# jinbeizame007/pytorch-r2d2-DPG

Measured on NVIDIA H100. Metric: learner sequence-steps/sec (batch x seq_len), higher is better.
Workload: dtype bf16x3 (fp32 operands split into bf16 hi+lo, three tensor-core passes, fp32 accumulate: ~16-bit operands)

## Files before the change

pytorch-r2d2-dpg_b200/csrc/lstm_scan.cu:

```cuda
#include <cooperative_groups.h>
#include <stdlib.h>

#include "gemm.cuh"
#include "lstm_scan.cuh"
#include "elementwise.cuh"
#include "sm90.cuh"

namespace cg = cooperative_groups;

namespace r2d2 {
namespace {

constexpr int SCAN_THREADS = 256;
constexpr int UNITS_PER_CTA = 32;
constexpr int ROWS_PER_CTA = 128;
constexpr int GT_LD = ROWS_PER_CTA + 4;
constexpr int DG_LD = ROWS_PER_CTA + 8;
constexpr unsigned long long kWaitLimitNs = 4000000000ull;

__device__ unsigned g_scan_status = 0;

__device__ __forceinline__ float accurate_sigmoid(float x) { return 1.0f / (1.0f + expf(-x)); }

__device__ __forceinline__ unsigned long long global_ns() {
  unsigned long long t;
  asm volatile("mov.u64 %0, %globaltimer;" : "=l"(t));
  return t;
}

__device__ __forceinline__ void wait_slice(uint64_t* bar, uint32_t parity) {
  if (sm90::mbar_try_wait(bar, parity)) return;
  if (*reinterpret_cast<volatile unsigned*>(&g_scan_status)) return;
  const unsigned long long t0 = global_ns();
  while (!sm90::mbar_try_wait(bar, parity)) {
    if (global_ns() - t0 > kWaitLimitNs) {
      atomicExch(&g_scan_status, 1u);
      return;
    }
  }
}

__device__ __forceinline__ uint32_t slice_parity(int s) { return (uint32_t)((s - 1) >> 1) & 1u; }

template <int H> __host__ __device__ constexpr bool w_hi_in_smem() { return H > 256; }

template <int H, int NB>
struct FwdSmem {
  static constexpr int C = H / 32;
  static constexpr int HROW = UNITS_PER_CTA + 8;
  static constexpr int SLICE = 2 * NB * HROW;
  static constexpr int W_BYTES = w_hi_in_smem<H>() ? (H / 16) * 8 * 32 * 16 : 0;
  static constexpr int HB_ELEMS = 2 * C * SLICE;
  static constexpr int GT_ELEMS = NB * GT_LD;
  static constexpr int HS_ELEMS = SLICE;
  static constexpr int BAR_OFF = W_BYTES + HB_ELEMS * 2 + GT_ELEMS * 4 + HS_ELEMS * 2;
  static constexpr int BYTES = BAR_OFF + 2 * C * 8;
  static_assert((SLICE * 2) % 16 == 0 && BAR_OFF % 16 == 0, "bulk copies need 16-byte granules");
  static_assert(BYTES <= 232448, "forward scan tile does not fit in 227 KB of shared memory");
};

template <int H, int NB>
__global__ void __launch_bounds__(SCAN_THREADS, 1) lstm_scan_fwd_kernel(ScanFwdParams p) {
  constexpr int C = H / 32, KS = H / 16, NT = NB / 8;
  constexpr bool WS = w_hi_in_smem<H>();
  using SM = FwdSmem<H, NB>;
  constexpr int HROW = SM::HROW, SLICE = SM::SLICE;
  cg::cluster_group cluster = cg::this_cluster();
  const int rank = (int)cluster.block_rank();
  const int b0 = (blockIdx.x / C) * NB;
  const int tid = threadIdx.x, lane = tid & 31, w = tid >> 5;
  const int g = lane >> 2, c = lane & 3;
  const int B = p.B, S = p.T * p.repeat;

  extern __shared__ __align__(16) unsigned char smem_raw[];
  uint4* w_hi_s = reinterpret_cast<uint4*>(smem_raw);
  __nv_bfloat16* hb = reinterpret_cast<__nv_bfloat16*>(smem_raw + SM::W_BYTES);
  float* gt = reinterpret_cast<float*>(smem_raw + SM::W_BYTES + SM::HB_ELEMS * 2);
  __nv_bfloat16* hstage = reinterpret_cast<__nv_bfloat16*>(smem_raw + SM::W_BYTES + SM::HB_ELEMS * 2 + SM::GT_ELEMS * 4);
  uint64_t* bar = reinterpret_cast<uint64_t*>(smem_raw + SM::BAR_OFF);

  for (int idx = tid; idx < NB * H; idx += SCAN_THREADS) {
    const int n = idx / H, k = idx % H, b = b0 + n;
    float v = (b < B && p.h0) ? __ldg(p.h0 + (size_t)b * H + k) : 0.f;
    __nv_bfloat16 hi, lo;
    split_bf16(v, hi, lo);
    __nv_bfloat16* row = hb + (0 * C + k / UNITS_PER_CTA) * SLICE + n * HROW + k % UNITS_PER_CTA;
    row[0] = hi;
    row[NB * HROW] = lo;
  }
  const int ug = rank * 32 + lane;
  float cst[NT];
#pragma unroll
  for (int e = 0; e < NT; ++e) {
    const int b = b0 + w + 8 * e;
    cst[e] = 0.f;
    if (b < B) {
      float hv = p.h0 ? __ldg(p.h0 + (size_t)b * H + ug) : 0.f;
      float cv = p.c0 ? __ldg(p.c0 + (size_t)b * H + ug) : 0.f;
      p.hs[(size_t)b * H + ug] = hv;
      p.cs[(size_t)b * H + ug] = cv;
      cst[e] = cv;
    }
  }
  if (tid < 2 * C) {
    sm90::mbar_init(bar + tid, 1);
    sm90::fence_mbar_init_cluster();
    sm90::mbar_arrive_expect_tx(bar + tid, SLICE * 2);
  }

  uint32_t a_hi[WS ? 1 : KS][4], a_lo[KS][4];
  {
    const int gate = w >> 1;
    const int u_lo = (w & 1) * 16 + g;
    const float* w_r0 = p.whh + (size_t)(gate * H + rank * 32 + u_lo) * H;
    const float* w_r1 = w_r0 + (size_t)8 * H;
#pragma unroll
    for (int ks = 0; ks < KS; ++ks) {
      const int k = ks * 16 + 2 * c;
      float2 v0 = __ldg(reinterpret_cast<const float2*>(w_r0 + k));
      float2 v1 = __ldg(reinterpret_cast<const float2*>(w_r1 + k));
      float2 v2 = __ldg(reinterpret_cast<const float2*>(w_r0 + k + 8));
      float2 v3 = __ldg(reinterpret_cast<const float2*>(w_r1 + k + 8));
      uint32_t h[4];
      split_pack2(v0.x, v0.y, h[0], a_lo[ks][0]);
      split_pack2(v1.x, v1.y, h[1], a_lo[ks][1]);
      split_pack2(v2.x, v2.y, h[2], a_lo[ks][2]);
      split_pack2(v3.x, v3.y, h[3], a_lo[ks][3]);
      if constexpr (WS) {
        w_hi_s[(ks * 8 + w) * 32 + lane] = make_uint4(h[0], h[1], h[2], h[3]);
      } else {
#pragma unroll
        for (int f = 0; f < 4; ++f) a_hi[ks][f] = h[f];
      }
    }
  }
  __syncthreads();
  cluster.sync();

  const size_t gstride = (size_t)4 * H;
  for (int s = 0; s < S; ++s) {
    const int cur = s & 1, nxt = cur ^ 1;
    const int t = s / p.repeat;

#pragma unroll
    for (int nt = 0; nt < NT; ++nt)
#pragma unroll
      for (int f = 0; f < 4; ++f) {
        const int n = nt * 8 + 2 * c + (f & 1), r = 16 * w + g + (f >> 1) * 8, b = b0 + n;
        if (b < B) sm90::cp_async_4(gt + n * GT_LD + r, p.gin + ((size_t)t * B + b) * gstride + (r >> 5) * H + rank * 32 + (r & 31));
      }
    sm90::cp_async_commit();

    float acc[NT][4];
#pragma unroll
    for (int nt = 0; nt < NT; ++nt)
#pragma unroll
      for (int e = 0; e < 4; ++e) acc[nt][e] = 0.f;
    const __nv_bfloat16* hb_cur = hb + cur * C * SLICE;
    uint64_t* bar_cur = bar + cur * C;
    const uint32_t parity = slice_parity(s);
#pragma unroll
    for (int ks = 0; ks < KS; ++ks) {
      if ((ks & 1) == 0 && s > 0) wait_slice(bar_cur + ks / 2, parity);
      const __nv_bfloat16* hb_hi = hb_cur + (ks / 2) * SLICE;
      const __nv_bfloat16* hb_lo = hb_hi + NB * HROW;
      uint32_t ah[4];
      if constexpr (WS) {
        const uint4 v = w_hi_s[(ks * 8 + w) * 32 + lane];
        ah[0] = v.x; ah[1] = v.y; ah[2] = v.z; ah[3] = v.w;
      } else {
#pragma unroll
        for (int f = 0; f < 4; ++f) ah[f] = a_hi[ks][f];
      }
#pragma unroll
      for (int nt = 0; nt < NT; ++nt) {
        const int off = (nt * 8 + g) * HROW + (ks & 1) * 16 + 2 * c;
        uint32_t bh[2], bl[2];
        bh[0] = *reinterpret_cast<const uint32_t*>(hb_hi + off);
        bh[1] = *reinterpret_cast<const uint32_t*>(hb_hi + off + 8);
        bl[0] = *reinterpret_cast<const uint32_t*>(hb_lo + off);
        bl[1] = *reinterpret_cast<const uint32_t*>(hb_lo + off + 8);
        mma_bf16_16816(acc[nt], a_lo[ks], bh);
        mma_bf16_16816(acc[nt], ah, bl);
        mma_bf16_16816(acc[nt], ah, bh);
      }
    }
    sm90::cp_async_wait_all();
#pragma unroll
    for (int nt = 0; nt < NT; ++nt) {
      const int n = nt * 8 + 2 * c, r = 16 * w + g;
      gt[n * GT_LD + r] += acc[nt][0];
      gt[(n + 1) * GT_LD + r] += acc[nt][1];
      gt[n * GT_LD + r + 8] += acc[nt][2];
      gt[(n + 1) * GT_LD + r + 8] += acc[nt][3];
    }
    if (w == 0 && lane < C) sm90::bulk_wait_read_all();
    __syncthreads();
    if (s > 0 && tid < C) sm90::mbar_arrive_expect_tx(bar_cur + tid, SLICE * 2);

#pragma unroll
    for (int e = 0; e < NT; ++e) {
      const int n = w + 8 * e, b = b0 + n;
      __nv_bfloat16 hi = __float2bfloat16_rn(0.f), lo = hi;
      if (b < B) {
        const float* gr = gt + n * GT_LD + lane;
        const float ig = accurate_sigmoid(gr[0]);
        const float fg = accurate_sigmoid(gr[32]);
        const float gg = tanhf(gr[64]);
        const float og = accurate_sigmoid(gr[96]);
        const float cn = fg * cst[e] + ig * gg;
        const float hn = og * tanhf(cn);
        cst[e] = cn;
        if (!p.no_save) {
          float* go = p.gates + ((size_t)s * B + b) * gstride + ug;
          go[0] = ig; go[H] = fg; go[2 * H] = gg; go[3 * H] = og;
          p.cs[((size_t)(s + 1) * B + b) * H + ug] = cn;
        }
        p.hs[((size_t)(s + 1) * B + b) * H + ug] = hn;
        if (p.head_in && (s % p.repeat) == p.repeat - 1)
          p.head_in[((size_t)t * B + b) * H + ug] = tanhf(hn);
        split_bf16(hn, hi, lo);
      }
      hstage[(0 * NB + n) * HROW + lane] = hi;
      hstage[(1 * NB + n) * HROW + lane] = lo;
    }
    sm90::fence_proxy_async_smem();
    __syncthreads();

    if (s + 1 < S && w == 0 && lane < C) {
      const uint32_t slot = sm90::smem_u32(hb + (nxt * C + rank) * SLICE);
      const uint32_t slot_bar = sm90::smem_u32(bar + nxt * C + rank);
      sm90::bulk_copy_s2cluster(sm90::map_cluster(slot, lane), sm90::smem_u32(hstage), SLICE * 2,
                                sm90::map_cluster(slot_bar, lane));
      sm90::bulk_commit();
    }
  }
  cluster.sync();
}

template <int H, int NB>
struct BwdSmem {
  static constexpr int C = H / 32;
  static constexpr int DG_ELEMS = 2 * NB * DG_LD;
  static constexpr int PS_LD = NB + 2;
  static constexpr int PS_ELEMS = 2 * C * UNITS_PER_CTA * PS_LD;
  static constexpr int PS_BYTES_PER_SRC = UNITS_PER_CTA * NB * 4;
  static constexpr int MT = (H / 16 + 7) / 8;
  static constexpr int W_BYTES = w_hi_in_smem<H>() ? MT * 8 * 8 * 32 * 16 : 0;
  static constexpr int STAGE_PLANES = 6;
  static constexpr int STAGE_ELEMS = STAGE_PLANES * NB * UNITS_PER_CTA;
  static constexpr int BAR_OFF = W_BYTES + DG_ELEMS * 2 + PS_ELEMS * 4 + STAGE_ELEMS * 4;
  static constexpr int BYTES = BAR_OFF + 2 * C * 8;
  static_assert(BAR_OFF % 8 == 0, "mbarrier alignment");
  static_assert(BYTES <= 232448, "BPTT scan tile does not fit in 227 KB of shared memory");
};

template <int H, int NB>
__global__ void __launch_bounds__(SCAN_THREADS, 1) lstm_scan_bwd_kernel(ScanBwdParams p) {
  constexpr int C = H / 32, NT = NB / 8;
  constexpr int M_TILES = H / 16;
  constexpr int MT = (M_TILES + 7) / 8;
  constexpr int KS = ROWS_PER_CTA / 16;
  constexpr bool WS = w_hi_in_smem<H>();
  using SM = BwdSmem<H, NB>;
  cg::cluster_group cluster = cg::this_cluster();
  const int rank = (int)cluster.block_rank();
  const int b0 = (blockIdx.x / C) * NB;
  const int tid = threadIdx.x, lane = tid & 31, w = tid >> 5;
  const int g = lane >> 2, c = lane & 3;
  const int B = p.B, S = p.T * p.repeat;

  extern __shared__ __align__(16) unsigned char smem_raw[];
  uint4* w_hi_s = reinterpret_cast<uint4*>(smem_raw);
  __nv_bfloat16* dgs = reinterpret_cast<__nv_bfloat16*>(smem_raw + SM::W_BYTES);
  float* ps = reinterpret_cast<float*>(smem_raw + SM::W_BYTES + SM::DG_ELEMS * 2);
  float* stage = ps + SM::PS_ELEMS;
  uint64_t* bar = reinterpret_cast<uint64_t*>(smem_raw + SM::BAR_OFF);
  constexpr int PLANE = NB * UNITS_PER_CTA;
  constexpr size_t gstride = (size_t)4 * H;

  auto head_step = [&](int s) {
    const int rel = s - p.head_first_step;
    return p.dh_head && rel >= 0 && (rel % p.repeat) == p.repeat - 1;
  };
  auto prefetch = [&](int s) {
    const int rel = s - p.head_first_step;
    const bool head = head_step(s);
    unsigned tv;
    asm volatile("mov.u32 %0, %%tid.x;" : "=r"(tv));
    const int lane = tv & 31, w = tv >> 5, ug = rank * 32 + lane;
#pragma unroll
    for (int e = 0; e < NT; ++e) {
      const int n = w + 8 * e, b = b0 + n;
      if (b < B) {
        float* st = stage + n * UNITS_PER_CTA + lane;
        const float* gs = p.gates + ((size_t)s * B + b) * gstride + ug;
#pragma unroll
        for (int q = 0; q < 4; ++q) sm90::cp_async_4(st + q * PLANE, gs + q * H);
        sm90::cp_async_4(st + 4 * PLANE, p.cs + ((size_t)s * B + b) * H + ug);
        if (head) sm90::cp_async_4(st + 5 * PLANE, p.dh_head + ((size_t)(rel / p.repeat) * B + b) * H + ug);
      }
    }
    sm90::cp_async_commit();
  };

  if (tid < 2 * C) {
    sm90::mbar_init(bar + tid, 1);
    sm90::fence_mbar_init_cluster();
    sm90::mbar_arrive_expect_tx(bar + tid, SM::PS_BYTES_PER_SRC);
  }
  prefetch(S - 1);

  const float* w_t = p.whh + (size_t)(rank * 32 + 2 * c) * H + w * MT * 16 + g;
  uint32_t a_hi[WS ? 1 : MT][WS ? 1 : KS][4], a_lo[MT][KS][4];
#pragma unroll
  for (int i = 0; i < MT; ++i) {
    const int mi = w * MT + i;
#pragma unroll
    for (int ks = 0; ks < KS; ++ks) {
      uint32_t h[4];
#pragma unroll
      for (int f = 0; f < 4; ++f) {
        float v0 = 0.f, v1 = 0.f;
        if (mi < M_TILES) {
          const float* w0 = w_t + ((ks >> 1) * H + (ks & 1) * 16 + (f >> 1) * 8) * H + i * 16 + (f & 1) * 8;
          v0 = __ldg(w0);
          v1 = __ldg(w0 + H);
        }
        split_pack2(v0, v1, h[f], a_lo[i][ks][f]);
      }
      if constexpr (WS) {
        w_hi_s[((i * KS + ks) * 8 + w) * 32 + lane] = make_uint4(h[0], h[1], h[2], h[3]);
      } else {
#pragma unroll
        for (int f = 0; f < 4; ++f) a_hi[i][ks][f] = h[f];
      }
    }
  }

  __syncthreads();
  const int ug = rank * 32 + lane;
  float dcn[NT], keep[NT][4], c_new[NT];
#pragma unroll
  for (int e = 0; e < NT; ++e) {
    const int b = b0 + w + 8 * e;
    dcn[e] = 0.f;
    c_new[e] = b < B ? __ldg(p.cs + ((size_t)S * B + b) * H + ug) : 0.f;
#pragma unroll
    for (int q = 0; q < 4; ++q) keep[e][q] = 0.f;
  }
  cluster.sync();

  for (int it = 0; it < S; ++it) {
    const int s = S - 1 - it;
    const int buf = it & 1;
    const int t = s / p.repeat;
    const bool has_head = head_step(s);

    float dh_rec[NT];
#pragma unroll
    for (int e = 0; e < NT; ++e) dh_rec[e] = 0.f;
    if (it > 0) {
      const uint32_t parity = slice_parity(it);
#pragma unroll
      for (int src = 0; src < C; ++src) {
        wait_slice(bar + buf * C + src, parity);
        const float* pr = ps + ((buf * C + src) * UNITS_PER_CTA + lane) * SM::PS_LD + w;
#pragma unroll
        for (int e = 0; e < NT; ++e) dh_rec[e] += pr[8 * e];
      }
    }
    sm90::cp_async_wait_all();

#pragma unroll
    for (int e = 0; e < NT; ++e) {
      const int n = w + 8 * e, b = b0 + n;
      float dg[4] = {0.f, 0.f, 0.f, 0.f};
      if (b < B) {
        const float* st = stage + n * UNITS_PER_CTA + lane;
        float dh = dh_rec[e];
        if (has_head) dh += st[5 * PLANE];
        const float ig = st[0], fg = st[PLANE], gg = st[2 * PLANE], og = st[3 * PLANE];
        const float c_prev = st[4 * PLANE];
        const float tc = tanhf(c_new[e]);
        c_new[e] = c_prev;
        const float dc = dcn[e] + dh * og * (1.f - tc * tc);
        dg[3] = dh * tc * og * (1.f - og);
        dg[0] = dc * gg * ig * (1.f - ig);
        dg[1] = dc * c_prev * fg * (1.f - fg);
        dg[2] = dc * ig * (1.f - gg * gg);
        dcn[e] = dc * fg;
        float* go = p.dgates + ((size_t)s * B + b) * gstride + ug;
        go[0] = dg[0]; go[H] = dg[1]; go[2 * H] = dg[2]; go[3 * H] = dg[3];
        if (p.repeat > 1) {
#pragma unroll
          for (int q = 0; q < 4; ++q) keep[e][q] += dg[q];
          if (s % p.repeat == 0) {
            float* gi = p.dgin + ((size_t)t * B + b) * gstride + ug;
#pragma unroll
            for (int q = 0; q < 4; ++q) { gi[q * H] = keep[e][q]; keep[e][q] = 0.f; }
          }
        }
      }
#pragma unroll
      for (int q = 0; q < 4; ++q) {
        __nv_bfloat16 hi, lo;
        split_bf16(dg[q], hi, lo);
        dgs[(0 * NB + n) * DG_LD + q * 32 + lane] = hi;
        dgs[(1 * NB + n) * DG_LD + q * 32 + lane] = lo;
      }
    }
    __syncthreads();
    if (it > 0 && tid < C) sm90::mbar_arrive_expect_tx(bar + buf * C + tid, SM::PS_BYTES_PER_SRC);

    if (s > 0) {
      prefetch(s - 1);
      float acc[MT][NT][4];
#pragma unroll
      for (int i = 0; i < MT; ++i)
#pragma unroll
        for (int nt = 0; nt < NT; ++nt)
#pragma unroll
          for (int e = 0; e < 4; ++e) acc[i][nt][e] = 0.f;
      const __nv_bfloat16* d_hi = dgs;
      const __nv_bfloat16* d_lo = dgs + NB * DG_LD;
#pragma unroll
      for (int ks = 0; ks < KS; ++ks) {
        uint32_t bh[NT][2], bl[NT][2];
#pragma unroll
        for (int nt = 0; nt < NT; ++nt) {
          const int off = (nt * 8 + g) * DG_LD + ks * 16 + 2 * c;
          bh[nt][0] = *reinterpret_cast<const uint32_t*>(d_hi + off);
          bh[nt][1] = *reinterpret_cast<const uint32_t*>(d_hi + off + 8);
          bl[nt][0] = *reinterpret_cast<const uint32_t*>(d_lo + off);
          bl[nt][1] = *reinterpret_cast<const uint32_t*>(d_lo + off + 8);
        }
#pragma unroll
        for (int i = 0; i < MT; ++i) {
          uint32_t ah[4];
          if constexpr (WS) {
            const uint4 v = w_hi_s[((i * KS + ks) * 8 + w) * 32 + lane];
            ah[0] = v.x; ah[1] = v.y; ah[2] = v.z; ah[3] = v.w;
          } else {
#pragma unroll
            for (int f = 0; f < 4; ++f) ah[f] = a_hi[i][ks][f];
          }
#pragma unroll
          for (int nt = 0; nt < NT; ++nt) {
            mma_bf16_16816(acc[i][nt], a_lo[i][ks], bh[nt]);
            mma_bf16_16816(acc[i][nt], ah, bl[nt]);
            mma_bf16_16816(acc[i][nt], ah, bh[nt]);
          }
        }
      }
      const uint32_t slot_bar = sm90::smem_u32(bar + (buf ^ 1) * C + rank);
#pragma unroll
      for (int i = 0; i < MT; ++i) {
        const int mi = w * MT + i;
        if (mi < M_TILES) {
#pragma unroll
          for (int h2 = 0; h2 < 2; ++h2) {
            const int j = mi * 16 + g + h2 * 8;
            const int owner = j >> 5, jl = j & 31;
            const uint32_t slot = sm90::map_cluster(
                sm90::smem_u32(ps + (((buf ^ 1) * C + rank) * UNITS_PER_CTA + jl) * SM::PS_LD), owner);
            const uint32_t owner_bar = sm90::map_cluster(slot_bar, owner);
#pragma unroll
            for (int nt = 0; nt < NT; ++nt)
              sm90::st_async_f2(slot + (nt * 8 + 2 * c) * 4, acc[i][nt][2 * h2], acc[i][nt][2 * h2 + 1], owner_bar);
          }
        }
      }
    }
    __syncthreads();
  }
  cluster.sync();
}

__global__ void lstm_cell_fwd_pointwise(const float* __restrict__ gpre, const float* __restrict__ c_prev,
                                        float* __restrict__ gates, float* __restrict__ h_out,
                                        float* __restrict__ c_out, float* __restrict__ head_in, int B, int H) {
  const int idx = blockIdx.x * blockDim.x + threadIdx.x;
  if (idx >= B * H) return;
  const int b = idx / H, u = idx % H;
  const float* gr = gpre + (size_t)b * 4 * H + u;
  const float ig = accurate_sigmoid(gr[0]), fg = accurate_sigmoid(gr[H]);
  const float gg = tanhf(gr[2 * H]), og = accurate_sigmoid(gr[3 * H]);
  const float cn = fg * c_prev[idx] + ig * gg;
  const float hn = og * tanhf(cn);
  float* go = gates + (size_t)b * 4 * H + u;
  go[0] = ig; go[H] = fg; go[2 * H] = gg; go[3 * H] = og;
  h_out[idx] = hn;
  c_out[idx] = cn;
  if (head_in) head_in[idx] = tanhf(hn);
}

__global__ void lstm_cell_bwd_pointwise(const float* __restrict__ gates, const float* __restrict__ c_prev,
                                        const float* __restrict__ c_new, const float* __restrict__ dh_head,
                                        const float* __restrict__ dh_rec, float* __restrict__ dc_state,
                                        float* __restrict__ dgates, float* __restrict__ dgin, int dgin_mode,
                                        int B, int H) {
  const int idx = blockIdx.x * blockDim.x + threadIdx.x;
  if (idx >= B * H) return;
  const int b = idx / H, u = idx % H;
  const float* gs = gates + (size_t)b * 4 * H + u;
  const float ig = gs[0], fg = gs[H], gg = gs[2 * H], og = gs[3 * H];
  float dh = dh_rec ? dh_rec[idx] : 0.f;
  if (dh_head) dh += dh_head[idx];
  const float tc = tanhf(c_new[idx]);
  const float dc = dc_state[idx] + dh * og * (1.f - tc * tc);
  float dg[4];
  dg[3] = dh * tc * og * (1.f - og);
  dg[0] = dc * gg * ig * (1.f - ig);
  dg[1] = dc * c_prev[idx] * fg * (1.f - fg);
  dg[2] = dc * ig * (1.f - gg * gg);
  dc_state[idx] = dc * fg;
  float* go = dgates + (size_t)b * 4 * H + u;
  float* gi = dgin ? dgin + (size_t)b * 4 * H + u : nullptr;
#pragma unroll
  for (int q = 0; q < 4; ++q) {
    go[q * H] = dg[q];
    if (dgin_mode == 1) gi[q * H] = dg[q];
    else if (dgin_mode == 2) gi[q * H] += dg[q];
  }
}

int scan_forward_generic(const ScanFwdParams& p, float* scratch, cudaStream_t stream) {
  const int B = p.B, H = p.H, S = p.T * p.repeat;
  const size_t bh = (size_t)B * H;
  R2D2_REQUIRE(scratch != nullptr, "generic scan needs scratch");
  if (p.h0) R2D2_CUDA_TRY(cudaMemcpyAsync(p.hs, p.h0, bh * 4, cudaMemcpyDeviceToDevice, stream));
  else R2D2_CUDA_TRY(cudaMemsetAsync(p.hs, 0, bh * 4, stream));
  if (p.c0) R2D2_CUDA_TRY(cudaMemcpyAsync(p.cs, p.c0, bh * 4, cudaMemcpyDeviceToDevice, stream));
  else R2D2_CUDA_TRY(cudaMemsetAsync(p.cs, 0, bh * 4, stream));
  const int blocks = ceil_div((int)bh, 256);
  for (int s = 0; s < S; ++s) {
    const int t = s / p.repeat;
    GemmParams g;
    g.A = p.hs + (size_t)s * bh; g.lda = H;
    g.B = p.whh; g.ldb = H;
    g.C = scratch; g.ldc = 4 * H;
    g.M = B; g.N = 4 * H; g.K = H;
    g.Z = p.gin + (size_t)t * B * 4 * H; g.ldz = 4 * H;
    g.epilogue = EPI_ADD_Z;
    R2D2_TRY(gemm_f32(g, GEMM_NT, stream));
    float* head = (p.head_in && (s % p.repeat) == p.repeat - 1) ? p.head_in + (size_t)t * bh : nullptr;
    lstm_cell_fwd_pointwise<<<blocks, 256, 0, stream>>>(scratch, p.cs + (size_t)s * bh,
                                                         p.gates + (size_t)s * B * 4 * H, p.hs + (size_t)(s + 1) * bh,
                                                         p.cs + (size_t)(s + 1) * bh, head, B, H);
    count_launch();
  }
  R2D2_CUDA_TRY(cudaGetLastError());
  return R2D2_OK;
}

int scan_backward_generic(const ScanBwdParams& p, cudaStream_t stream) {
  const int B = p.B, H = p.H, S = p.T * p.repeat;
  const size_t bh = (size_t)B * H;
  R2D2_REQUIRE(p.scratch != nullptr, "generic scan needs scratch");
  float* dh_rec = p.scratch;
  float* dc_state = p.scratch + bh;
  R2D2_CUDA_TRY(cudaMemsetAsync(p.scratch, 0, 2 * bh * 4, stream));
  const int blocks = ceil_div((int)bh, 256);
  for (int s = S - 1; s >= 0; --s) {
    const int t = s / p.repeat;
    const int rel = s - p.head_first_step;
    const bool has_head = p.dh_head && rel >= 0 && (rel % p.repeat) == p.repeat - 1;
    const float* head = has_head ? p.dh_head + (size_t)(rel / p.repeat) * bh : nullptr;
    int mode = 0;
    if (p.repeat > 1) mode = ((s % p.repeat) == p.repeat - 1) ? 1 : 2;
    lstm_cell_bwd_pointwise<<<blocks, 256, 0, stream>>>(
        p.gates + (size_t)s * B * 4 * H, p.cs + (size_t)s * bh, p.cs + (size_t)(s + 1) * bh, head,
        (s == S - 1) ? nullptr : dh_rec, dc_state, p.dgates + (size_t)s * B * 4 * H,
        mode ? p.dgin + (size_t)t * B * 4 * H : nullptr, mode, B, H);
    count_launch();
    if (s > 0) {
      GemmParams g;
      g.A = p.dgates + (size_t)s * B * 4 * H; g.lda = 4 * H;
      g.B = p.whh; g.ldb = H;
      g.C = dh_rec; g.ldc = H;
      g.M = B; g.N = H; g.K = 4 * H;
      R2D2_TRY(gemm_f32(g, GEMM_NN, stream));
    }
  }
  R2D2_CUDA_TRY(cudaGetLastError());
  return R2D2_OK;
}

template <typename Kern>
int set_cluster_attributes(Kern kern, int cluster_size, int smem_bytes) {
  R2D2_CUDA_TRY(cudaFuncSetAttribute(kern, cudaFuncAttributeMaxDynamicSharedMemorySize, smem_bytes));
  if (cluster_size > 8) R2D2_CUDA_TRY(cudaFuncSetAttribute(kern, cudaFuncAttributeNonPortableClusterSizeAllowed, 1));
  return R2D2_OK;
}

cudaLaunchConfig_t cluster_config(int cluster_size, int n_clusters, int smem_bytes, cudaStream_t stream,
                                  cudaLaunchAttribute* attr) {
  cudaLaunchConfig_t cfg = {};
  cfg.gridDim = dim3(cluster_size * n_clusters);
  cfg.blockDim = dim3(SCAN_THREADS);
  cfg.dynamicSmemBytes = smem_bytes;
  cfg.stream = stream;
  attr[0].id = cudaLaunchAttributeClusterDimension;
  attr[0].val.clusterDim.x = cluster_size;
  attr[0].val.clusterDim.y = 1;
  attr[0].val.clusterDim.z = 1;
  cfg.attrs = attr;
  cfg.numAttrs = 1;
  return cfg;
}

template <typename Kern, typename Params>
int launch_cluster(Kern kern, const Params& p, int cluster_size, int n_clusters, int smem_bytes, cudaStream_t stream) {
  R2D2_TRY(set_cluster_attributes(kern, cluster_size, smem_bytes));
  cudaLaunchAttribute attr[1];
  cudaLaunchConfig_t cfg = cluster_config(cluster_size, n_clusters, smem_bytes, stream, attr);
  R2D2_CUDA_TRY(cudaLaunchKernelEx(&cfg, kern, p));
  count_launch();
  return R2D2_OK;
}

template <typename Kern>
int resident_clusters(Kern kern, int cluster_size, int smem_bytes, int* out) {
  R2D2_TRY(set_cluster_attributes(kern, cluster_size, smem_bytes));
  cudaLaunchAttribute attr[1];
  cudaLaunchConfig_t cfg = cluster_config(cluster_size, 1, smem_bytes, nullptr, attr);
  R2D2_CUDA_TRY(cudaOccupancyMaxActiveClusters(out, kern, &cfg));
  return R2D2_OK;
}

template <int H, typename K8, typename K16, typename K32>
int pick_nb(int B, K8 k8, int smem8, K16 k16, int smem16, K32 k32, int smem32, int* nb) {
  int fit = 0;
  R2D2_TRY(resident_clusters(k8, H / 32, smem8, &fit));
  if (ceil_div(B, 8) <= fit) { *nb = 8; return R2D2_OK; }
  R2D2_TRY(resident_clusters(k16, H / 32, smem16, &fit));
  if (ceil_div(B, 16) <= fit || !k32) { *nb = 16; return R2D2_OK; }
  *nb = 32;
  (void)smem32;
  return R2D2_OK;
}

template <int H>
int fwd_dispatch(const ScanFwdParams& p, cudaStream_t stream) {
  constexpr bool WIDE = !w_hi_in_smem<H>();
  constexpr int NB3 = WIDE ? 32 : 16;
  int nb = 0;
  R2D2_TRY(pick_nb<H>(p.B, lstm_scan_fwd_kernel<H, 8>, FwdSmem<H, 8>::BYTES, lstm_scan_fwd_kernel<H, 16>,
                      FwdSmem<H, 16>::BYTES, WIDE ? lstm_scan_fwd_kernel<H, NB3> : nullptr, FwdSmem<H, NB3>::BYTES, &nb));
  if (nb == 8)
    return launch_cluster(lstm_scan_fwd_kernel<H, 8>, p, H / 32, ceil_div(p.B, 8), FwdSmem<H, 8>::BYTES, stream);
  if (nb == 16)
    return launch_cluster(lstm_scan_fwd_kernel<H, 16>, p, H / 32, ceil_div(p.B, 16), FwdSmem<H, 16>::BYTES, stream);
  return launch_cluster(lstm_scan_fwd_kernel<H, NB3>, p, H / 32, ceil_div(p.B, NB3), FwdSmem<H, NB3>::BYTES, stream);
}
template <int H>
int bwd_dispatch(const ScanBwdParams& p, cudaStream_t stream) {
  constexpr bool WIDE = !w_hi_in_smem<H>();
  constexpr int NB3 = WIDE ? 32 : 16;
  int nb = 0;
  R2D2_TRY(pick_nb<H>(p.B, lstm_scan_bwd_kernel<H, 8>, BwdSmem<H, 8>::BYTES, lstm_scan_bwd_kernel<H, 16>,
                      BwdSmem<H, 16>::BYTES, WIDE ? lstm_scan_bwd_kernel<H, NB3> : nullptr, BwdSmem<H, NB3>::BYTES, &nb));
  if (nb == 8)
    return launch_cluster(lstm_scan_bwd_kernel<H, 8>, p, H / 32, ceil_div(p.B, 8), BwdSmem<H, 8>::BYTES, stream);
  if (nb == 16)
    return launch_cluster(lstm_scan_bwd_kernel<H, 16>, p, H / 32, ceil_div(p.B, 16), BwdSmem<H, 16>::BYTES, stream);
  return launch_cluster(lstm_scan_bwd_kernel<H, NB3>, p, H / 32, ceil_div(p.B, NB3), BwdSmem<H, NB3>::BYTES, stream);
}

}

bool lstm_scan_cluster_supported(int H) { return H == 32 || H == 64 || H == 128 || H == 256 || H == 512; }

static int g_scan_impl = -1;
void lstm_scan_set_impl(int impl) { g_scan_impl = impl ? 1 : 0; }
int lstm_scan_get_impl() {
  if (g_scan_impl < 0) {
    const char* e = getenv("R2D2_SCAN_IMPL");
    g_scan_impl = (e && (e[0] == 's' || e[0] == '0')) ? 0 : 1;
  }
  return g_scan_impl;
}
static bool use_cluster_kernels(int H) { return lstm_scan_cluster_supported(H) && lstm_scan_get_impl() == 1; }

int lstm_scan_error_status(int* out, cudaStream_t stream) {
  R2D2_REQUIRE(out, "null");
  unsigned v = 0;
  R2D2_CUDA_TRY(cudaMemcpyFromSymbolAsync(&v, g_scan_status, sizeof(v), 0, cudaMemcpyDeviceToHost, stream));
  R2D2_CUDA_TRY(cudaStreamSynchronize(stream));
  *out = (int)v;
  return R2D2_OK;
}

size_t lstm_scan_fwd_scratch_floats(int B, int H) { return (size_t)B * 4 * H; }
size_t lstm_scan_bwd_scratch_floats(int B, int H) { return (size_t)2 * B * H; }

int lstm_scan_forward(const ScanFwdParams& p, cudaStream_t stream) {
  R2D2_REQUIRE(p.gin && p.whh && p.gates && p.hs && p.cs, "null pointer");
  R2D2_REQUIRE(p.T > 0 && p.B > 0 && p.H > 0 && p.repeat >= 1, "shape");
  R2D2_REQUIRE(p.repeat == 1 || p.gates != p.gin, "gates must not alias gin when repeat > 1");
  if (use_cluster_kernels(p.H)) {
    switch (p.H) {
      case 32: return fwd_dispatch<32>(p, stream);
      case 64: return fwd_dispatch<64>(p, stream);
      case 128: return fwd_dispatch<128>(p, stream);
      case 256: return fwd_dispatch<256>(p, stream);
      case 512: return fwd_dispatch<512>(p, stream);
      default: break;
    }
  }
  return scan_forward_generic(p, p.scratch, stream);
}

int lstm_scan_backward(const ScanBwdParams& p, cudaStream_t stream) {
  R2D2_REQUIRE(p.gates && p.hs && p.cs && p.whh && p.dgates, "null pointer");
  R2D2_REQUIRE(p.T > 0 && p.B > 0 && p.H > 0 && p.repeat >= 1, "shape");
  R2D2_REQUIRE(p.repeat == 1 || (p.dgin && p.dgin != p.dgates), "dgin buffer required when repeat > 1");
  int rc = R2D2_OK;
  switch (use_cluster_kernels(p.H) ? p.H : 0) {
    case 32: rc = bwd_dispatch<32>(p, stream); break;
    case 64: rc = bwd_dispatch<64>(p, stream); break;
    case 128: rc = bwd_dispatch<128>(p, stream); break;
    case 256: rc = bwd_dispatch<256>(p, stream); break;
    case 512: rc = bwd_dispatch<512>(p, stream); break;
    default: rc = scan_backward_generic(p, stream); break;
  }
  R2D2_TRY(rc);
  if (p.dbias) {
    const float* src = p.repeat > 1 ? p.dgin : p.dgates;
    R2D2_TRY(colsum(src, 4 * p.H, p.T * p.B, 4 * p.H, p.dbias, p.dbias2, stream));
  }
  return R2D2_OK;
}

}
```

pytorch-r2d2-dpg_b200/csrc/lstm_scan.cuh:

```cuda
#pragma once
#include "common.cuh"

namespace r2d2 {

struct ScanFwdParams {
  const float* gin = nullptr;
  const float* whh = nullptr;
  const float* h0 = nullptr;
  const float* c0 = nullptr;
  float* gates = nullptr;
  float* hs = nullptr;
  float* cs = nullptr;
  float* head_in = nullptr;
  int T = 0, B = 0, H = 0, repeat = 1;
  float* scratch = nullptr;
  int no_save = 0;
};

struct ScanBwdParams {
  const float* gates = nullptr;
  const float* hs = nullptr;
  const float* cs = nullptr;
  const float* whh = nullptr;
  const float* dh_head = nullptr;
  int head_first_step = 0;
  float* dgates = nullptr;
  float* dgin = nullptr;
  int T = 0, B = 0, H = 0, repeat = 1;
  float* scratch = nullptr;
  float* dbias = nullptr;
  float* dbias2 = nullptr;
};

bool lstm_scan_cluster_supported(int H);
int lstm_scan_forward(const ScanFwdParams& p, cudaStream_t stream);
int lstm_scan_backward(const ScanBwdParams& p, cudaStream_t stream);
size_t lstm_scan_fwd_scratch_floats(int B, int H);
size_t lstm_scan_bwd_scratch_floats(int B, int H);

void lstm_scan_set_impl(int impl);
int lstm_scan_get_impl();
int lstm_scan_error_status(int* out, cudaStream_t stream);

}
```

pytorch-r2d2-dpg_b200/csrc/sm90.cuh:

```cuda
#pragma once
#include <cuda_runtime.h>
#include <stdint.h>

namespace r2d2 {
namespace sm90 {

__device__ __forceinline__ uint32_t smem_u32(const void* p) { return (uint32_t)__cvta_generic_to_shared(p); }

__device__ __forceinline__ uint64_t make_smem_desc(uint32_t smem_addr, uint32_t lbo_bytes, uint32_t sbo_bytes) {
  uint64_t d = 0;
  d |= (uint64_t)((smem_addr >> 4) & 0x3FFF);
  d |= (uint64_t)((lbo_bytes >> 4) & 0x3FFF) << 16;
  d |= (uint64_t)((sbo_bytes >> 4) & 0x3FFF) << 32;
  return d;
}

__device__ __forceinline__ void wgmma_fence() { asm volatile("wgmma.fence.sync.aligned;" ::: "memory"); }
__device__ __forceinline__ void wgmma_commit() { asm volatile("wgmma.commit_group.sync.aligned;" ::: "memory"); }
template <int N>
__device__ __forceinline__ void wgmma_wait() { asm volatile("wgmma.wait_group.sync.aligned %0;" ::"n"(N) : "memory"); }
__device__ __forceinline__ void fence_regs(float (&d)[64]) {
#pragma unroll
  for (int i = 0; i < 64; ++i) asm volatile("" : "+f"(d[i])::"memory");
}

template <int TA, int TB>
__device__ __forceinline__ void wgmma_m64n128k16_bf16(float (&d)[64], uint64_t da, uint64_t db) {
  asm volatile(
      "{\n\t"
      ".reg .pred p;\n\t"
      "setp.ne.b32 p, 1, 0;\n\t"
      "wgmma.mma_async.sync.aligned.m64n128k16.f32.bf16.bf16 "
      "{%0,%1,%2,%3,%4,%5,%6,%7,%8,%9,%10,%11,%12,%13,%14,%15,"
      "%16,%17,%18,%19,%20,%21,%22,%23,%24,%25,%26,%27,%28,%29,%30,%31,"
      "%32,%33,%34,%35,%36,%37,%38,%39,%40,%41,%42,%43,%44,%45,%46,%47,"
      "%48,%49,%50,%51,%52,%53,%54,%55,%56,%57,%58,%59,%60,%61,%62,%63}, "
      "%64, %65, p, 1, 1, %66, %67;\n\t"
      "}\n"
      : "+f"(d[0]), "+f"(d[1]), "+f"(d[2]), "+f"(d[3]), "+f"(d[4]), "+f"(d[5]), "+f"(d[6]), "+f"(d[7]),
        "+f"(d[8]), "+f"(d[9]), "+f"(d[10]), "+f"(d[11]), "+f"(d[12]), "+f"(d[13]), "+f"(d[14]), "+f"(d[15]),
        "+f"(d[16]), "+f"(d[17]), "+f"(d[18]), "+f"(d[19]), "+f"(d[20]), "+f"(d[21]), "+f"(d[22]), "+f"(d[23]),
        "+f"(d[24]), "+f"(d[25]), "+f"(d[26]), "+f"(d[27]), "+f"(d[28]), "+f"(d[29]), "+f"(d[30]), "+f"(d[31]),
        "+f"(d[32]), "+f"(d[33]), "+f"(d[34]), "+f"(d[35]), "+f"(d[36]), "+f"(d[37]), "+f"(d[38]), "+f"(d[39]),
        "+f"(d[40]), "+f"(d[41]), "+f"(d[42]), "+f"(d[43]), "+f"(d[44]), "+f"(d[45]), "+f"(d[46]), "+f"(d[47]),
        "+f"(d[48]), "+f"(d[49]), "+f"(d[50]), "+f"(d[51]), "+f"(d[52]), "+f"(d[53]), "+f"(d[54]), "+f"(d[55]),
        "+f"(d[56]), "+f"(d[57]), "+f"(d[58]), "+f"(d[59]), "+f"(d[60]), "+f"(d[61]), "+f"(d[62]), "+f"(d[63])
      : "l"(da), "l"(db), "n"(TA), "n"(TB));
}

__device__ __forceinline__ float ex2_approx(float x) { float y; asm("ex2.approx.ftz.f32 %0, %1;" : "=f"(y) : "f"(x)); return y; }
__device__ __forceinline__ float rcp_approx(float x) { float y; asm("rcp.approx.ftz.f32 %0, %1;" : "=f"(y) : "f"(x)); return y; }
__device__ __forceinline__ float tanh_fast(float x) { return 2.0f * rcp_approx(1.0f + ex2_approx(-2.8853900817779268f * x)) - 1.0f; }

__device__ __forceinline__ bool elect_one() {
  uint32_t pred;
  asm volatile(
      "{\n\t"
      ".reg .pred p;\n\t"
      "elect.sync _|p, 0xffffffff;\n\t"
      "selp.u32 %0, 1, 0, p;\n\t"
      "}\n"
      : "=r"(pred));
  return pred != 0;
}

__device__ __forceinline__ void mbar_init(uint64_t* bar, uint32_t count) {
  asm volatile("mbarrier.init.shared::cta.b64 [%0], %1;" ::"r"(smem_u32(bar)), "r"(count) : "memory");
}
__device__ __forceinline__ void mbar_arrive(uint64_t* bar) {
  asm volatile("mbarrier.arrive.shared::cta.b64 _, [%0];" ::"r"(smem_u32(bar)) : "memory");
}
__device__ __forceinline__ void mbar_arrive_expect_tx(uint64_t* bar, uint32_t tx_bytes) {
  asm volatile("mbarrier.arrive.expect_tx.shared::cta.b64 _, [%0], %1;" ::"r"(smem_u32(bar)), "r"(tx_bytes) : "memory");
}
__device__ __forceinline__ bool mbar_try_wait(uint64_t* bar, uint32_t parity) {
  uint32_t ok;
  asm volatile(
      "{\n\t"
      ".reg .pred p;\n\t"
      "mbarrier.try_wait.parity.shared::cta.b64 p, [%1], %2;\n\t"
      "selp.u32 %0, 1, 0, p;\n\t"
      "}\n"
      : "=r"(ok)
      : "r"(smem_u32(bar)), "r"(parity)
      : "memory");
  return ok != 0;
}

__device__ __forceinline__ void bulk_copy_g2s(uint32_t dst_smem_addr, const void* src_global, uint32_t bytes, uint32_t mbar_smem_addr) {
  asm volatile("cp.async.bulk.shared::cluster.global.mbarrier::complete_tx::bytes [%0], [%1], %2, [%3];" ::"r"(dst_smem_addr),
               "l"(src_global), "r"(bytes), "r"(mbar_smem_addr)
               : "memory");
}

__device__ __forceinline__ void cp_async_4(float* smem_dst, const float* gsrc) {
  asm volatile("cp.async.ca.shared.global [%0], [%1], 4;" ::"r"((uint32_t)__cvta_generic_to_shared(smem_dst)), "l"(gsrc) : "memory");
}
__device__ __forceinline__ void cp_async_commit() { asm volatile("cp.async.commit_group;" ::: "memory"); }
__device__ __forceinline__ void cp_async_wait_all() { asm volatile("cp.async.wait_group 0;" ::: "memory"); }

__device__ __forceinline__ void fence_mbar_init_cluster() { asm volatile("fence.mbarrier_init.release.cluster;" ::: "memory"); }
__device__ __forceinline__ void fence_proxy_async_smem() { asm volatile("fence.proxy.async.shared::cta;" ::: "memory"); }
__device__ __forceinline__ uint32_t map_cluster(uint32_t smem_addr, uint32_t rank) {
  uint32_t r;
  asm volatile("mapa.shared::cluster.u32 %0, %1, %2;" : "=r"(r) : "r"(smem_addr), "r"(rank));
  return r;
}
__device__ __forceinline__ void bulk_copy_s2cluster(uint32_t dst_cluster_addr, uint32_t src_smem_addr, uint32_t bytes,
                                                    uint32_t mbar_cluster_addr) {
  asm volatile("cp.async.bulk.shared::cluster.shared::cta.mbarrier::complete_tx::bytes [%0], [%1], %2, [%3];"
               ::"r"(dst_cluster_addr), "r"(src_smem_addr), "r"(bytes), "r"(mbar_cluster_addr)
               : "memory");
}
__device__ __forceinline__ void bulk_commit() { asm volatile("cp.async.bulk.commit_group;" ::: "memory"); }
__device__ __forceinline__ void bulk_wait_read_all() { asm volatile("cp.async.bulk.wait_group.read 0;" ::: "memory"); }
__device__ __forceinline__ void st_async_f2(uint32_t dst_cluster_addr, float x, float y, uint32_t mbar_cluster_addr) {
  asm volatile("st.async.shared::cluster.mbarrier::complete_tx::bytes.v2.f32 [%0], {%1, %2}, [%3];"
               ::"r"(dst_cluster_addr), "f"(x), "f"(y), "r"(mbar_cluster_addr)
               : "memory");
}

}
}
```

Baseline: 1.113 million.

## Single-buffer hidden-state exchange for wide-H NB=32 scan and split batch launches

For large hidden sizes with 32-row tiles, the forward LSTM scan drops the double-buffered hidden-state slices and the separate staging buffer. Each CTA writes its own slice in place, and peers signal through remote mbarrier arrivals before a slice is overwritten. This shrinks shared memory enough that the NB=32 variant fits with the weights held in smem. The dispatcher then launches full waves of NB=32 clusters and covers the remainder with a second launch offset by a new row0 parameter. The cost is a stricter handshake that can stall a producer until all consumers have read, plus an extra kernel launch.

```diff
diff --git a/pytorch-r2d2-dpg_b200/csrc/lstm_scan.cu b/pytorch-r2d2-dpg_b200/csrc/lstm_scan.cu
--- a/pytorch-r2d2-dpg_b200/csrc/lstm_scan.cu
+++ b/pytorch-r2d2-dpg_b200/csrc/lstm_scan.cu
@@ -46,13 +46,14 @@
 
 template <int H, int NB>
 struct FwdSmem {
+  static constexpr bool SB = w_hi_in_smem<H>() && NB > 16;
   static constexpr int C = H / 32;
   static constexpr int HROW = UNITS_PER_CTA + 8;
   static constexpr int SLICE = 2 * NB * HROW;
   static constexpr int W_BYTES = w_hi_in_smem<H>() ? (H / 16) * 8 * 32 * 16 : 0;
-  static constexpr int HB_ELEMS = 2 * C * SLICE;
+  static constexpr int HB_ELEMS = (SB ? 1 : 2) * C * SLICE;
   static constexpr int GT_ELEMS = NB * GT_LD;
-  static constexpr int HS_ELEMS = SLICE;
+  static constexpr int HS_ELEMS = SB ? 0 : SLICE;
   static constexpr int BAR_OFF = W_BYTES + HB_ELEMS * 2 + GT_ELEMS * 4 + HS_ELEMS * 2;
   static constexpr int BYTES = BAR_OFF + 2 * C * 8;
   static_assert((SLICE * 2) % 16 == 0 && BAR_OFF % 16 == 0, "bulk copies need 16-byte granules");
@@ -64,10 +65,11 @@
   constexpr int C = H / 32, KS = H / 16, NT = NB / 8;
   constexpr bool WS = w_hi_in_smem<H>();
   using SM = FwdSmem<H, NB>;
+  constexpr bool SB = SM::SB;
   constexpr int HROW = SM::HROW, SLICE = SM::SLICE;
   cg::cluster_group cluster = cg::this_cluster();
   const int rank = (int)cluster.block_rank();
-  const int b0 = (blockIdx.x / C) * NB;
+  const int b0 = p.row0 + (blockIdx.x / C) * NB;
   const int tid = threadIdx.x, lane = tid & 31, w = tid >> 5;
   const int g = lane >> 2, c = lane & 3;
   const int B = p.B, S = p.T * p.repeat;
@@ -76,7 +78,8 @@
   uint4* w_hi_s = reinterpret_cast<uint4*>(smem_raw);
   __nv_bfloat16* hb = reinterpret_cast<__nv_bfloat16*>(smem_raw + SM::W_BYTES);
   float* gt = reinterpret_cast<float*>(smem_raw + SM::W_BYTES + SM::HB_ELEMS * 2);
-  __nv_bfloat16* hstage = reinterpret_cast<__nv_bfloat16*>(smem_raw + SM::W_BYTES + SM::HB_ELEMS * 2 + SM::GT_ELEMS * 4);
+  __nv_bfloat16* hstage = SB ? hb + rank * SLICE
+                             : reinterpret_cast<__nv_bfloat16*>(smem_raw + SM::W_BYTES + SM::HB_ELEMS * 2 + SM::GT_ELEMS * 4);
   uint64_t* bar = reinterpret_cast<uint64_t*>(smem_raw + SM::BAR_OFF);
 
   for (int idx = tid; idx < NB * H; idx += SCAN_THREADS) {
@@ -105,7 +108,7 @@
   if (tid < 2 * C) {
     sm90::mbar_init(bar + tid, 1);
     sm90::fence_mbar_init_cluster();
-    sm90::mbar_arrive_expect_tx(bar + tid, SLICE * 2);
+    if (!SB || (tid < C && tid != rank)) sm90::mbar_arrive_expect_tx(bar + tid, SLICE * 2);
   }
 
   uint32_t a_hi[WS ? 1 : KS][4], a_lo[KS][4];
@@ -139,7 +142,7 @@
 
   const size_t gstride = (size_t)4 * H;
   for (int s = 0; s < S; ++s) {
-    const int cur = s & 1, nxt = cur ^ 1;
+    const int cur = SB ? 0 : s & 1, nxt = SB ? 0 : cur ^ 1;
     const int t = s / p.repeat;
 
 #pragma unroll
@@ -158,10 +161,10 @@
       for (int e = 0; e < 4; ++e) acc[nt][e] = 0.f;
     const __nv_bfloat16* hb_cur = hb + cur * C * SLICE;
     uint64_t* bar_cur = bar + cur * C;
-    const uint32_t parity = slice_parity(s);
+    const uint32_t parity = SB ? (uint32_t)(s - 1) & 1u : slice_parity(s);
 #pragma unroll
     for (int ks = 0; ks < KS; ++ks) {
-      if ((ks & 1) == 0 && s > 0) wait_slice(bar_cur + ks / 2, parity);
+      if ((ks & 1) == 0 && s > 0 && (!SB || ks / 2 != rank)) wait_slice(bar_cur + ks / 2, parity);
       const __nv_bfloat16* hb_hi = hb_cur + (ks / 2) * SLICE;
       const __nv_bfloat16* hb_lo = hb_hi + NB * HROW;
       uint32_t ah[4];
@@ -196,7 +199,9 @@
     }
     if (w == 0 && lane < C) sm90::bulk_wait_read_all();
     __syncthreads();
-    if (s > 0 && tid < C) sm90::mbar_arrive_expect_tx(bar_cur + tid, SLICE * 2);
+    if (s > 0 && tid < C && (!SB || tid != rank)) sm90::mbar_arrive_expect_tx(bar_cur + tid, SLICE * 2);
+    if (SB && s + 1 < S && tid < C && tid != rank)
+      sm90::mbar_arrive_remote(sm90::map_cluster(sm90::smem_u32(bar + C + rank), tid));
 
 #pragma unroll
     for (int e = 0; e < NT; ++e) {
@@ -227,7 +232,8 @@
     sm90::fence_proxy_async_smem();
     __syncthreads();
 
-    if (s + 1 < S && w == 0 && lane < C) {
+    if (s + 1 < S && w == 0 && lane < C && (!SB || lane != rank)) {
+      if (SB) wait_slice(bar + C + lane, (uint32_t)s & 1u);
       const uint32_t slot = sm90::smem_u32(hb + (nxt * C + rank) * SLICE);
       const uint32_t slot_bar = sm90::smem_u32(bar + nxt * C + rank);
       sm90::bulk_copy_s2cluster(sm90::map_cluster(slot, lane), sm90::smem_u32(hstage), SLICE * 2,
@@ -642,17 +648,35 @@
 }
 
 template <int H>
+int fwd_launch(const ScanFwdParams& p, int rows, cudaStream_t stream) {
+  int nb = 0;
+  R2D2_TRY(pick_nb<H>(rows, lstm_scan_fwd_kernel<H, 8>, FwdSmem<H, 8>::BYTES, lstm_scan_fwd_kernel<H, 16>,
+                      FwdSmem<H, 16>::BYTES, lstm_scan_fwd_kernel<H, 32>, FwdSmem<H, 32>::BYTES, &nb));
+  if (nb == 8)
+    return launch_cluster(lstm_scan_fwd_kernel<H, 8>, p, H / 32, ceil_div(rows, 8), FwdSmem<H, 8>::BYTES, stream);
+  if (nb == 16)
+    return launch_cluster(lstm_scan_fwd_kernel<H, 16>, p, H / 32, ceil_div(rows, 16), FwdSmem<H, 16>::BYTES, stream);
+  return launch_cluster(lstm_scan_fwd_kernel<H, 32>, p, H / 32, ceil_div(rows, 32), FwdSmem<H, 32>::BYTES, stream);
+}
+
+template <int H>
 int fwd_dispatch(const ScanFwdParams& p, cudaStream_t stream) {
-  constexpr bool WIDE = !w_hi_in_smem<H>();
-  constexpr int NB3 = WIDE ? 32 : 16;
-  int nb = 0;
-  R2D2_TRY(pick_nb<H>(p.B, lstm_scan_fwd_kernel<H, 8>, FwdSmem<H, 8>::BYTES, lstm_scan_fwd_kernel<H, 16>,
-                      FwdSmem<H, 16>::BYTES, WIDE ? lstm_scan_fwd_kernel<H, NB3> : nullptr, FwdSmem<H, NB3>::BYTES, &nb));
-  if (nb == 8)
-    return launch_cluster(lstm_scan_fwd_kernel<H, 8>, p, H / 32, ceil_div(p.B, 8), FwdSmem<H, 8>::BYTES, stream);
-  if (nb == 16)
-    return launch_cluster(lstm_scan_fwd_kernel<H, 16>, p, H / 32, ceil_div(p.B, 16), FwdSmem<H, 16>::BYTES, stream);
-  return launch_cluster(lstm_scan_fwd_kernel<H, NB3>, p, H / 32, ceil_div(p.B, NB3), FwdSmem<H, NB3>::BYTES, stream);
+  if constexpr (w_hi_in_smem<H>()) {
+    int fit16 = 0, fit32 = 0;
+    R2D2_TRY(resident_clusters(lstm_scan_fwd_kernel<H, 16>, H / 32, FwdSmem<H, 16>::BYTES, &fit16));
+    R2D2_TRY(resident_clusters(lstm_scan_fwd_kernel<H, 32>, H / 32, FwdSmem<H, 32>::BYTES, &fit32));
+    const int wave = 32 * fit32;
+    const int covered = wave > 0 ? (p.B / wave) * wave : 0;
+    const int rest = p.B - covered;
+    if (p.B > 16 * fit16 && covered > 0 && rest <= 16 * fit16) {
+      R2D2_TRY(launch_cluster(lstm_scan_fwd_kernel<H, 32>, p, H / 32, covered / 32, FwdSmem<H, 32>::BYTES, stream));
+      if (rest == 0) return R2D2_OK;
+      ScanFwdParams q = p;
+      q.row0 = covered;
+      return fwd_launch<H>(q, rest, stream);
+    }
+  }
+  return fwd_launch<H>(p, p.B, stream);
 }
 template <int H>
 int bwd_dispatch(const ScanBwdParams& p, cudaStream_t stream) {
diff --git a/pytorch-r2d2-dpg_b200/csrc/lstm_scan.cuh b/pytorch-r2d2-dpg_b200/csrc/lstm_scan.cuh
--- a/pytorch-r2d2-dpg_b200/csrc/lstm_scan.cuh
+++ b/pytorch-r2d2-dpg_b200/csrc/lstm_scan.cuh
@@ -15,6 +15,7 @@
   int T = 0, B = 0, H = 0, repeat = 1;
   float* scratch = nullptr;
   int no_save = 0;
+  int row0 = 0;
 };
 
 struct ScanBwdParams {
diff --git a/pytorch-r2d2-dpg_b200/csrc/sm90.cuh b/pytorch-r2d2-dpg_b200/csrc/sm90.cuh
--- a/pytorch-r2d2-dpg_b200/csrc/sm90.cuh
+++ b/pytorch-r2d2-dpg_b200/csrc/sm90.cuh
@@ -70,6 +70,9 @@
 __device__ __forceinline__ void mbar_arrive(uint64_t* bar) {
   asm volatile("mbarrier.arrive.shared::cta.b64 _, [%0];" ::"r"(smem_u32(bar)) : "memory");
 }
+__device__ __forceinline__ void mbar_arrive_remote(uint32_t mbar_cluster_addr) {
+  asm volatile("mbarrier.arrive.release.cta.shared::cluster.b64 _, [%0];" ::"r"(mbar_cluster_addr) : "memory");
+}
 __device__ __forceinline__ void mbar_arrive_expect_tx(uint64_t* bar, uint32_t tx_bytes) {
   asm volatile("mbarrier.arrive.expect_tx.shared::cta.b64 _, [%0], %1;" ::"r"(smem_u32(bar)), "r"(tx_bytes) : "memory");
 }
```

Measured after the change: 1.137 million, median of 6. 2.2% higher.
